# gyhandy/Neural-Sim-NeRF

Hardware: AMD Instinct MI355X
Metric: Mray-samples/sec at 400x400, 64+128 samples, 8x256 MLP (higher is better)
Workload: dtype f16x2

## Files before the change

### neural_sim_nerf_amd/csrc/nsr_kernels.hip

```cpp
#include <hip/hip_runtime.h>
#include <stdint.h>
#include "nsr_device.h"

#if !defined(NSR_UNIT_F32) && !defined(NSR_UNIT_H2) && !defined(NSR_UNIT_B3) && !defined(NSR_UNIT_X16)
#define NSR_UNIT_F32 1
#define NSR_UNIT_H2 1
#define NSR_UNIT_B3 1
#define NSR_UNIT_X16 1
#endif
#ifndef NSR_UNIT_F32
#define NSR_UNIT_F32 0
#endif
#ifndef NSR_UNIT_H2
#define NSR_UNIT_H2 0
#endif
#ifndef NSR_UNIT_B3
#define NSR_UNIT_B3 0
#endif
#ifndef NSR_UNIT_X16
#define NSR_UNIT_X16 0
#endif
#define NSR_CAT_(a, b) a##b
#define NSR_CAT(a, b) NSR_CAT_(a, b)

// ... 70 lines not shown
  rg.pslot = __builtin_amdgcn_readfirstlane(rg.pslot);
  rg.pphase = __builtin_amdgcn_readfirstlane(rg.pphase);
  rg.cslot = __builtin_amdgcn_readfirstlane(rg.cslot);
  rg.pnet_off = __builtin_amdgcn_readfirstlane(rg.pnet_off);
  rg.pnet_next = __builtin_amdgcn_readfirstlane(rg.pnet_next);
}

#ifndef NSR_H2_SCHED
#define NSR_H2_SCHED 3
#endif
constexpr int kH2RingLag = NSR_H2_SCHED == 3 ? 1 : 0;
template <int NS = kRingSlots, int SLABS = kStreamSlabs, int SLABS_BWD = SLABS, int LAG = 0>
__device__ __forceinline__ void ring_start(Ring& rg, f32x4 (&A0)[4], int lane) {
#pragma unroll 1
  for (int s = 0; s < NS - LAG; ++s) ring_issue<NS, SLABS, SLABS_BWD>(rg);
  asm volatile("s_waitcnt vmcnt(%0)" ::"n"(4 * (NS - LAG - 1)) : "memory");
  __builtin_amdgcn_s_barrier();
  const char* p = rg.smem + rg.cslot * kSlabBytes + lane * 16;
#pragma unroll
  for (int c = 0; c < 4; ++c) A0[c] = *(const f32x4*)(p + c * 1024);
}

template <int U>
__device__ __forceinline__ void ring_load_quarter(const Ring& rg, f32x4 (&A)[4], int lane) {
  const char* p = rg.smem + rg.cslot * kSlabBytes + U * kStepBytes + lane * 16;
#pragma unroll
  for (int c = 0; c < 4; ++c) A[c] = *(const f32x4*)(p + c * 1024);
}

template <int NS = kRingSlots>
__device__ __forceinline__ void ring_advance(Ring& rg, f32x4 (&A)[4], int lane) {
  asm volatile("s_waitcnt vmcnt(%0) lgkmcnt(0)" ::"n"(4 * (NS - 2)) : "memory");
#ifndef NSR_EXP_NOBARRIER
  __builtin_amdgcn_s_barrier();
#endif
  rg.cslot = (rg.cslot + 1 == NS) ? 0 : rg.cslot + 1;
  const char* p = rg.smem + rg.cslot * kSlabBytes + lane * 16;
#pragma unroll
  for (int c = 0; c < 4; ++c) A[c] = *(const f32x4*)(p + c * 1024);
}

#define NSR_MFMA(a, b, c) __builtin_amdgcn_mfma_f32_32x32x2f32((a), (b), (c), 0, 0, 0)
__device__ __forceinline__ f32x16 mfma_op(float a, float b, f32x16 c) { return __builtin_amdgcn_mfma_f32_32x32x2f32(a, b, c, 0, 0, 0); }
__device__ __forceinline__ f32x4 mfma_op(float a, float b, f32x4 c) { return __builtin_amdgcn_mfma_f32_16x16x4f32(a, b, c, 0, 0, 0); }

template <int NMO, int KK0, int KK1, bool ZERO = false, int NACC, typename BOp, typename AccT>
__device__ __forceinline__ void consume(const f32x4 (&A)[4], int step, BOp bop, AccT (&acc)[NACC]) {
#pragma unroll
  for (int kk = KK0; kk < KK1; ++kk)
#pragma unroll
    for (int c = 0; c < 4; ++c) {
      const int n = 4 * step + c, tq = n / NMO, mo = n % NMO;
      if (ZERO && tq == 0 && kk == 0) acc[mo] = mfma_op(A[c][kk], bop(4 * tq + kk), AccT{0});
      else acc[mo] = mfma_op(A[c][kk], bop(4 * tq + kk), acc[mo]);
    }
}

#define NSR_PIN() __builtin_amdgcn_sched_barrier(0)
#define NSR_SGB(mask, n) __builtin_amdgcn_sched_group_barrier((mask), (n), 0)
#define NSR_MASK_VALU 0x002
#define NSR_MASK_SALU 0x004
#define NSR_MASK_MFMA 0x008
#define NSR_MASK_VMEM 0x010
#define NSR_MASK_DSRD 0x100
template <int N_MFMA>
__device__ __forceinline__ void step_pattern() {
#pragma unroll
  for (int i = 0; i < N_MFMA; ++i) {
    NSR_SGB(NSR_MASK_MFMA, 1);
    NSR_SGB(NSR_MASK_DSRD, 1);
    NSR_SGB(NSR_MASK_VALU, 2);
  }
}
template <int N_MFMA>
__device__ __forceinline__ void step_pattern_dma() {
#pragma unroll
  for (int i = 0; i < N_MFMA; ++i) {
    NSR_SGB(NSR_MASK_MFMA, 1);
    NSR_SGB(NSR_MASK_DSRD, 1);
    NSR_SGB(NSR_MASK_VMEM, 1);
    NSR_SGB(NSR_MASK_SALU, 3);
    NSR_SGB(NSR_MASK_VALU, 2);
  }
}

template <int NMO, int NTQ, int NS = kRingSlots, bool ZERO = false, int NACC, typename BOp, typename AccT>
__device__ __forceinline__ void seg(Ring& rg, f32x4 (&A0)[4], f32x4 (&A1)[4], BOp bop, AccT (&acc)[NACC],
                                    int lane) {
  static_assert((NMO * NTQ) % 16 == 0, "a segment is a whole number of slabs");
#pragma unroll
  for (int s = 0; s < NMO * NTQ / 4; s += 4) {
    NSR_PIN(); ring_load_quarter<1>(rg, A1, lane); consume<NMO, 0, 4, ZERO>(A0, s, bop, acc);     step_pattern<16>();
    NSR_PIN(); ring_load_quarter<2>(rg, A0, lane); consume<NMO, 0, 4, ZERO>(A1, s + 1, bop, acc); step_pattern<16>();
    NSR_PIN(); ring_load_quarter<3>(rg, A1, lane); consume<NMO, 0, 4, ZERO>(A0, s + 2, bop, acc); step_pattern<16>();
    NSR_PIN(); consume<NMO, 0, 1, ZERO>(A1, s + 3, bop, acc);
    NSR_PIN(); ring_advance<NS>(rg, A0, lane);
    ring_issue<NS>(rg); consume<NMO, 1, 4, ZERO>(A1, s + 3, bop, acc); step_pattern_dma<12>();
    NSR_PIN();
  }
}

template <int NG>
struct BRegs16 {
  const f32x16 (&v)[NG];
  __device__ __forceinline__ float operator()(int t) const { return v[t >> 4][t & 15]; }
};
template <int N>
struct BArr {
  const float (&v)[N];
  __device__ __forceinline__ float operator()(int t) const { return v[t]; }
};
struct BViews {
  const f32x16 (&v)[8];
  const float (&ed)[16];
  __device__ __forceinline__ float operator()(int t) const { return t < 128 ? v[(t & 127) >> 4][t & 15] : ed[t & 15]; }
};

__device__ __forceinline__ int aux_half(int lane) { return opaque_v((lane >> 5) * 4); }

template <int NMO>
__device__ __forceinline__ void load_bias(const float* bias, int h4 , f32x16 (&acc)[NMO]) {
#pragma unroll
  for (int mo = 0; mo < NMO; ++mo)
#pragma unroll
    for (int rq = 0; rq < 4; ++rq) {
      f32x4 v = *(const f32x4*)(bias + (mo * 4 + rq) * 8 + h4);
      acc[mo][rq * 4 + 0] = v[0];
      acc[mo][rq * 4 + 1] = v[1];
      acc[mo][rq * 4 + 2] = v[2];
      acc[mo][rq * 4 + 3] = v[3];
    }
}

#include "nsr_b3.inc"
#include "nsr_h2.inc"

constexpr int kMlpF32 = 0;
constexpr int kMlpB3 = 1;
constexpr int kMlpH2 = 2;

template <int NMO>
__device__ __forceinline__ uint4 relu_mask(const f32x16 (&acc)[NMO]) {
  unsigned w[4] = {0u, 0u, 0u, 0u};
#pragma unroll
  for (int mo = 0; mo < NMO; ++mo)
#pragma unroll
    for (int r = 0; r < 16; ++r) {
      const int on = max(__float_as_int(acc[mo][r]), 0) - 1;
      w[mo >> 1] = __builtin_amdgcn_alignbit(w[mo >> 1], (unsigned)on, 31);
    }
  return make_uint4(w[0], w[1], w[2], w[3]);
}

__device__ __forceinline__ float enc_trig(float a, int k) {
  const double kMagic = 6755399441055744.0;
  const double t = (double)a * 0.63661977236758134308;
  const double tm = t + kMagic;
  const int n = __double2loint(tm) + k;
  const double f = t - (tm - kMagic);
  const float r = (float)(f * 1.57079632679489661923);
  const float z = r * r;
  float ps = __builtin_fmaf(-1.9515295891e-4f, z, 8.3321608736e-3f);
  ps = __builtin_fmaf(ps, z, -1.6666654611e-1f);
  ps = __builtin_fmaf(ps * z, r, r);
  float pc = __builtin_fmaf(2.443315711809948e-5f, z, -1.388731625493765e-3f);
  pc = __builtin_fmaf(pc, z, 4.166664568298827e-2f);
  pc = __builtin_fmaf(pc * z, z, __builtin_fmaf(-0.5f, z, 1.0f));
  const float v = (n & 1) ? pc : ps;
  return __uint_as_float(__float_as_uint(v) ^ ((unsigned)(n & 2) << 30));
}

__device__ __forceinline__ float enc_domain(float x, int nfreq) {
  return __builtin_fabsf(x) < ldexpf(1.0f, 25 - nfreq) ? x : __builtin_nanf("");
}

__device__ __forceinline__ float enc_poison(float px, float py, float pz, float vx, float vy, float vz) {
  const float a = (enc_domain(px, kMultires) * 0.0f + enc_domain(py, kMultires) * 0.0f) + enc_domain(pz, kMultires) * 0.0f;
  const float b = (enc_domain(vx, kMultiresViews) * 0.0f + enc_domain(vy, kMultiresViews) * 0.0f) +
                  enc_domain(vz, kMultiresViews) * 0.0f;
  return __builtin_fabsf(a + b);
}

template <bool CAPTURE, int MODE = kMlpF32>
__device__ __forceinline__ void mlp_pass(Ring& rg, const float* aux, f32x4 (&A0)[4], f32x4 (&A1)[4], int lane,
                                         float px, float py, float pz, float vx, float vy, float vz,
                                         float (&raw)[4], uint4* mask_dst = nullptr , int mask_tid = 0,
                                         long long* tp = nullptr ) {
#ifdef NSR_PHASE_TIMING
  long long tpl = clock64();
#define NSR_TP(i) do { if (tp) { const long long t_ = clock64(); tp[i] += t_ - tpl; tpl = t_; } } while (0)
#else
#define NSR_TP(i) do { } while (0)
#endif
  const int h = lane >> 5;
  const int h4 = aux_half(lane);
  const float poison = enc_poison(px, py, pz, vx, vy, vz);
  float e[32];
  float ed[16];
  {
    const float p[3] = {px, py, pz};
    const float v[3] = {vx, vy, vz};
#pragma unroll
    for (int L = 0; L < kMultires; ++L)
#pragma unroll
      for (int ax = 0; ax < 3; ++ax) e[3 * L + ax] = enc_trig(enc_domain(p[ax], kMultires) * (float)(1 << L), h);
#pragma unroll
    for (int L = 0; L < kMultiresViews; ++L)
#pragma unroll
      for (int ax = 0; ax < 3; ++ax) ed[3 * L + ax] = enc_trig(enc_domain(v[ax], kMultiresViews) * (float)(1 << L), h);
    e[30] = h ? pz : px;
    e[31] = h ? 0.0f : py;
    ed[12] = h ? vz : vx;
    ed[13] = h ? 0.0f : vy;
    ed[14] = 0.0f;
    ed[15] = 0.0f;
  }

  f32x16 acc[8];
  f32x16 in[8];
  auto enc_src = [&](int kb, int i) { return e[(8 * kb + i) & 31]; };
  auto in_src = [&](int kb, int i) { return in[(kb >> 1) & 7][8 * (kb & 1) + i]; };
  constexpr bool B3 = MODE == kMlpB3;
  constexpr bool H2M = MODE == kMlpH2;
  float amax = 0.0f;
  const float* h2s = aux + kAuxH2Scale;
#if NSR_H2_SCHED == 3 && !defined(NSR_EXP_H2_NOFRAG) && !defined(NSR_EXP_H2_HALFBARRIER) && !defined(NSR_EXP_H2_NOSPLIT)
  constexpr bool TAIL = H2M && !CAPTURE;
#else
  constexpr bool TAIL = false;
#endif
  static_assert(kAuxBiasV == kAuxBias + 9 * 256, "the views layer's bias follows feature_linear's: 'bias of layer L + 1' for L = 8");
  NSR_TP(0);
  load_bias<8>(aux + kAuxBias, h4, acc);
  NSR_TP(2);
  if constexpr (B3) gemm_b3<8, 2>(rg, A0, A1, enc_src, acc, lane);
  else if constexpr (TAIL)
    gemm_h2_tail<4>(rg, A0, A1, enc_src, H2Scale{{h2s[0], 0.0f}, 4}, acc, lane, amax, H2Tail{acc, in, 0, h2_lds_base(aux + kAuxBias + 256, h4)});
  else if constexpr (H2M) gemm_h2<8, 4>(rg, A0, A1, enc_src, H2Scale{{h2s[0], 0.0f}, 4}, acc, lane, amax);
  else seg<8, 8>(rg, A0, A1, BArr<32>{e}, acc, lane);
  NSR_TP(1);
  if (CAPTURE) mask_dst[mask_tid] = relu_mask<8>(acc);
  if constexpr (!TAIL) {
#pragma unroll
    for (int mo = 0; mo < 8; ++mo) in[mo] = relu16(acc[mo]);
  }

  float alpha_part = 0.0f;
#pragma unroll 1
  for (int L = 1; L <= 8; ++L) {
    if constexpr (!TAIL) load_bias<8>(aux + kAuxBias + L * 256, h4, acc);
    NSR_TP(2);
    if (L == 5) {
      if constexpr (B3) gemm_b3<8, 2>(rg, A0, A1, enc_src, acc, lane);
      else if constexpr (H2M) gemm_h2<8, 4>(rg, A0, A1, enc_src, H2Scale{{h2s[9], 0.0f}, 4}, acc, lane, amax);
      else seg<8, 8>(rg, A0, A1, BArr<32>{e}, acc, lane);
      NSR_TP(1);
    }
    if (L == 8) {
      const float* wa = aux + kAuxWAlpha;
#pragma unroll
      for (int tq = 0; tq < 32; ++tq) {
        f32x4 w = *(const f32x4*)(wa + tq * 8 + h4);
#pragma unroll
        for (int kk = 0; kk < 4; ++kk)
          alpha_part = __builtin_fmaf(w[kk], in[(4 * tq + kk) >> 4][(4 * tq + kk) & 15], alpha_part);
      }
    }
    if constexpr (B3) gemm_b3<8, 8>(rg, A0, A1, in_src, acc, lane);
    else if constexpr (TAIL)
      gemm_h2_tail<16>(rg, A0, A1, in_src, H2Scale{{h2s[L], 0.0f}, 16}, acc, lane, amax,
                       H2Tail{acc, in, (L == 8) ? (int)0x80000000 : 0, h2_lds_base(aux + kAuxBias + (L + 1) * 256, h4)});
    else if constexpr (H2M) gemm_h2<8, 16>(rg, A0, A1, in_src, H2Scale{{h2s[L], 0.0f}, 16}, acc, lane, amax);
    else seg<8, 32>(rg, A0, A1, BRegs16<8>{in}, acc, lane);
    NSR_TP(1);
    if (CAPTURE && L < 8) mask_dst[L * 256 + mask_tid] = relu_mask<8>(acc);
    if constexpr (!TAIL) {
      const int thr = (L == 8) ? (int)0x80000000 : 0;
#pragma unroll
      for (int mo = 0; mo < 8; ++mo) in[mo] = clamp_bits16(acc[mo], thr);
    }
  }

  f32x16 av[4];
  if constexpr (TAIL) {
#pragma unroll
    for (int mo = 0; mo < 4; ++mo) av[mo] = acc[mo];
  } else {
    load_bias<4>(aux + kAuxBiasV, h4, av);
  }
  NSR_TP(2);
  if constexpr (B3) {
    auto v_src = [&](int kb, int i) {
      return kb < 16 ? in[(kb >> 1) & 7][8 * (kb & 1) + i] : (kb < 18 ? ed[(8 * (kb - 16) + i) & 15] : 0.0f);
    };
    gemm_b3<4, 5>(rg, A0, A1, v_src, av, lane);
  } else if constexpr (H2M) {
    auto v_src = [&](int kb, int i) { return kb < 16 ? in[(kb >> 1) & 7][8 * (kb & 1) + i] : ed[(8 * (kb - 16) + i) & 15]; };
    gemm_h2<4, 18>(rg, A0, A1, v_src, H2Scale{{h2s[10], h2s[11]}, 16}, av, lane, amax);
  } else {
    seg<4, 36>(rg, A0, A1, BViews{in, ed}, av, lane);
  }
  NSR_TP(1);
  if (CAPTURE) mask_dst[8 * 256 + mask_tid] = relu_mask<4>(av);

  float part[4] = {0.0f, 0.0f, 0.0f, alpha_part};
  if constexpr (H2M) {
    const float ov = amax > kH2Max ? __builtin_nanf("") : 0.0f;
    part[0] = part[1] = part[2] = ov;
    part[3] = alpha_part + ov;
  }
#pragma unroll
  for (int c = 0; c < 3; ++c) {
    const float* wr = aux + kAuxWRgb + c * 128;
#pragma unroll
    for (int mo = 0; mo < 4; ++mo)
#pragma unroll
      for (int rq = 0; rq < 4; ++rq) {
        f32x4 w = *(const f32x4*)(wr + (mo * 4 + rq) * 8 + h4);
#pragma unroll
        for (int ri = 0; ri < 4; ++ri)
          part[c] = __builtin_fmaf(w[ri], fmaxf(av[mo][rq * 4 + ri], 0.0f), part[c]);
      }
  }
#pragma unroll
  for (int c = 0; c < 4; ++c) {
    float other = __shfl_xor(part[c], 32);
    float lo_half = h ? other : part[c];
    float hi_half = h ? part[c] : other;
    raw[c] = ((lo_half + hi_half) + aux[(c < 3) ? (kAuxBRgb + c) : kAuxBAlpha]) + poison;
  }
  NSR_TP(3);
#undef NSR_TP
}

template <int NSS, int NFS>
struct ItemStateT {
  static constexpr int kNS = NSS, kNF = NFS;
  float tcoarse[NSS];
  float ufine[128];
  float ray[2][16];
  float zc[2][NSS];
  float rawc[2][NSS][4];
  float w0[2][NSS];
  float cdf[2][NSS];
  float zs[2][128];
  float zf[2][NFS];
  float rawf[2][NFS][4];
  float alpha[2][NFS];
  float wf[2][NFS];
  float tf[2][NFS];
  float om[2][NFS];
  float bwd_scratch[2][NFS][2];
  float psum[2][NFS / 32][12];
  float gnorm[2];
  float res[2][8];
};
typedef ItemStateT<64, 192> ItemState;
typedef ItemStateT<128, 256> ItemStateBig;
static_assert(sizeof(ItemState) == 23048, "the YCB-V layout is part of the shipped kernels' LDS budget");
template <int NS> struct ItemStateFor { typedef ItemState type; };
template <> struct ItemStateFor<128> { typedef ItemStateBig type; };

__device__ __forceinline__ float sigmoidf_(float x) { return 1.0f / (1.0f + expf(-x)); }

template <int S, int R = 2, int STRIDE = S, typename ST>
__device__ __forceinline__ void composite(ST& st, const float* z, float* raw, float* wout, float* tout, int tid,
                                          const float* noise = nullptr ,
                                          long long row0 = 0, int valid = R) {
  static_assert(S % 8 == 0, "scan is unrolled by 8");
// ... 325 lines not shown
    __syncthreads();
  }
}

__device__ __forceinline__ void gen_ray(const float* __restrict__ c2w, float fx, float fy, float cx, float cy,
                                        int row, int col, float (&o)[3], float (&d)[3]) {
  const float dx = ((float)col - cx) / fx;
  const float dy = -(((float)row - cy) / fy);
  const float dz = -1.0f;
#pragma unroll
  for (int a = 0; a < 3; ++a) {
    d[a] = ((dx * c2w[a * 4 + 0]) + (dy * c2w[a * 4 + 1])) + (dz * c2w[a * 4 + 2]);
    o[a] = c2w[a * 4 + 3];
  }
}

struct RenderArgs {
  const float* nets;
  long long net_stride;
  const float* aux[2];
  const float* tcoarse;
  const float* ufine;
  const float* rays_o;
  const float* rays_d;
  const float* c2w;
  float fx, fy, cx, cy;
  int H, W;
  long long n_rays;
  float near_, far_;
  int fine;
  int camera;
  int white_bkgd;
  int lindisp;
  float *rgb, *disp, *acc, *rgb0, *disp0, *acc0, *z_std;
  float *dbg_w0, *dbg_zs, *dbg_zf, *dbg_raw0, *dbg_raw;
  long long* dbg_inds;
  float* zf_scratch;
  int chunk;
  unsigned* sched_flags;
  unsigned* status;
  int super_lg;
  int spin_max;
  unsigned epoch;
  unsigned* epoch_counter;
  unsigned long long* work_counter;
  const float* viewdirs;
  const float* t_rand;
  const float* u_rays;
  const float* noise0;
  const float* noise1;
  const float* near_rays;
  const float* far_rays;
  unsigned long long* ovf_items;
  unsigned* ovf_stat;
  unsigned ovf_cap;
  const unsigned long long* item_list;
  const unsigned* item_count;
  unsigned item_cap;
};

__device__ __forceinline__ void load_aux(char* smem, const RenderArgs& a, int tid) {
  float* dst = (float*)(smem + kLdsAux);
  for (int i = tid; i < kAuxFloats; i += 256) {
    dst[i] = a.aux[0][i];
    dst[kAuxFloats + i] = a.aux[1][i];
  }
}

#if NSR_UNIT_F32
__global__ void k_set_args(const RenderArgs a, RenderArgs* dst) {
  *dst = a;
  *a.work_counter = 0ull;
  if (a.ovf_stat) a.ovf_stat[0] = 0u;
  if (a.epoch_counter) dst->epoch = *a.epoch_counter = *a.epoch_counter % 4094u + 1u;
}
#endif

constexpr long long kItemMask = (1ll << 62) - 1;
__device__ __forceinline__ long long queue_next_item(const RenderArgs& q) {
  const unsigned long long v = atomicAdd(q.work_counter, 1ull);
  if (q.item_list) {
    unsigned n = *q.item_count;
    n = n < q.item_cap ? n : q.item_cap;
    return v < (unsigned long long)n ? (long long)q.item_list[v] : -1ll;
  }
  return v < (unsigned long long)((q.n_rays + 1) >> 1) ? (long long)(v | (3ull << 62)) : -1ll;
}
__device__ __forceinline__ long long queue_item_of(const RenderArgs& q, unsigned long long v) {
  if (q.item_list) {
    unsigned n = *q.item_count;
    n = n < q.item_cap ? n : q.item_cap;
    return v < (unsigned long long)n ? (long long)q.item_list[v] : -1ll;
  }
  return v < (unsigned long long)((q.n_rays + 1) >> 1) ? (long long)(v | (3ull << 62)) : -1ll;
}
__device__ __forceinline__ long long queue_items(const RenderArgs& q) {
  if (q.item_list) { const unsigned n = *q.item_count; return (long long)(n < q.item_cap ? n : q.item_cap); }
  return (q.n_rays + 1) >> 1;
}
__device__ __forceinline__ void range_mark(int* ovf, float chk, int lane) {
#ifndef NSR_EXP_NO_RANGE
  if (chk != chk && lane < 32) atomicAdd(ovf, 1);
#endif
}
__device__ __forceinline__ unsigned range_report(const RenderArgs& a, int* ovf, long long item, int valid) {
#ifdef NSR_EXP_NO_RANGE
  return 0u;
#endif
  const int p0 = ovf[0], p1 = valid == 2 ? ovf[1] : 0;
  if ((p0 | p1) != 0 && a.ovf_stat) {
    const unsigned long long mask = (p0 ? 1ull : 0ull) | (p1 ? 2ull : 0ull);
    const unsigned n = atomicAdd(a.ovf_stat, 1u);
    atomicAdd(a.ovf_stat + 1, (unsigned)(p0 + p1));
    if (n < a.ovf_cap) {
      a.ovf_items[n] = (unsigned long long)item | (mask << 62);
      atomicAdd(a.ovf_stat + 2, (unsigned)((p0 != 0) + (p1 != 0)));
    } else {
      atomicAdd(a.ovf_stat + 3, 1u);
      return (unsigned)mask;
    }
  }
  return 0u;
}
__device__ __forceinline__ void range_poison(const RenderArgs& a, long long ray0, unsigned mask) {
  const float qn = __builtin_nanf("");
  for (int r = 0; r < 2; ++r) {
    if (!((mask >> r) & 1u)) continue;
    const long long rr = ray0 + r;
    float* const v3[2] = {a.rgb, a.rgb0};
    float* const v1[5] = {a.disp, a.acc, a.disp0, a.acc0, a.z_std};
    for (int k = 0; k < 2; ++k) if (v3[k]) { v3[k][rr * 3] = qn; v3[k][rr * 3 + 1] = qn; v3[k][rr * 3 + 2] = qn; }
    for (int k = 0; k < 5; ++k) if (v1[k]) v1[k][rr] = qn;
  }
}

__device__ __forceinline__ void wave_lds_sync() {
  __builtin_amdgcn_fence(__ATOMIC_RELEASE, "wavefront");
  __builtin_amdgcn_wave_barrier();
  __builtin_amdgcn_fence(__ATOMIC_ACQUIRE, "wavefront");
}
__device__ __forceinline__ void lds_barrier() { asm volatile("s_waitcnt lgkmcnt(0)\n\ts_barrier" ::: "memory"); }

template <typename ST>
struct FwdItemExtra {
  float om[2][ST::kNS];
  float tf[2][ST::kNS];
  float zf[2][ST::kNF];
  float ray[2][16];
  float res[2][8];
  long long pend;
  long long next;
};

template <int S>
__device__ __forceinline__ void composite_wave(const float* ry, const float* zr, float* q, float* wr, float* tr, float* omr,
                                               int lane, const float* noise ,
                                               float (&res)[6]) {
  static_assert(S % 8 == 0, "scan is unrolled by 8");
  constexpr int K = (S + 63) / 64;
  float al[K];
#pragma unroll
  for (int k = 0; k < K; ++k) {
    const int i = lane + 64 * k;
    al[k] = 0.0f;
    if (i < S) {
      float dist = (i < S - 1) ? (zr[i + 1] - zr[i]) : 1e10f;
      dist = dist * ry[11];
      if (noise) q[i * 4 + 3] = q[i * 4 + 3] + noise[i];
      const float sigma = fmaxf(q[i * 4 + 3], 0.0f);
      const float a = 1.0f - expf(-sigma * dist);
      al[k] = a;
      omr[i] = (1.0f - a) + 1e-10f;
      q[i * 4 + 0] = sigmoidf_(q[i * 4 + 0]);
      q[i * 4 + 1] = sigmoidf_(q[i * 4 + 1]);
      q[i * 4 + 2] = sigmoidf_(q[i * 4 + 2]);
    }
  }
  wave_lds_sync();
  if (lane == 0) {
    double T = 1.0;
#pragma unroll 1
    for (int i0 = 0; i0 < S; i0 += 8) {
      double f[8];
#pragma unroll
      for (int k = 0; k < 8; ++k) f[k] = (double)omr[i0 + k];
#pragma unroll
      for (int k = 0; k < 8; ++k) {
        tr[i0 + k] = (float)T;
        T = T * f[k];
      }
    }
  }
  wave_lds_sync();
  float cr = 0.f, cg = 0.f, cb = 0.f, depth = 0.f, acc = 0.f;
#pragma unroll
  for (int k = 0; k < K; ++k) {
    const int i = lane + 64 * k;
    if (i < S) {
      const float w = al[k] * tr[i];
      wr[i] = w;
      cr = cr + w * q[i * 4 + 0];
      cg = cg + w * q[i * 4 + 1];
      cb = cb + w * q[i * 4 + 2];
      depth = depth + w * zr[i];
      acc = acc + w;
    }
  }
#pragma unroll
  for (int m = 32; m >= 1; m >>= 1) {
    cr += __shfl_xor(cr, m); cg += __shfl_xor(cg, m); cb += __shfl_xor(cb, m);
    depth += __shfl_xor(depth, m); acc += __shfl_xor(acc, m);
  }
  const float qd = depth / acc;
  float disp;
  if (qd != qd) disp = qd;
  else disp = 1.0f / fmaxf(1e-10f, qd);
  if (ry[12] != 0.0f) {
    const float bg = 1.0f - acc;
    cr = cr + bg; cg = cg + bg; cb = cb + bg;
  }
  res[0] = cr; res[1] = cg; res[2] = cb; res[3] = disp; res[4] = acc; res[5] = depth;
  wave_lds_sync();
}

template <int NI, int NS>
__device__ __forceinline__ void sample_pdf_wave(const float* w, const float* zc, float* x, float* pdf, float* cdf, float* zs,
                                                const float* u ,
                                                int64_t* inds_out , int lane) {
  constexpr int NW = NS - 2, NC = NS - 1;
  constexpr int NVEC = NW / 8, SILP = NVEC / 4;
  constexpr int KW = (NW + 63) / 64;
  float xv[KW];
#pragma unroll
  for (int k = 0; k < KW; ++k) {
    const int i = lane + 64 * k;
    xv[k] = 0.0f;
    if (i < NW) { xv[k] = w[i] + 1e-5f; x[i] = xv[k]; }
  }
  wave_lds_sync();
  const int j = lane & 7;
  float lj;
  if constexpr (NS == 64) {
    const float p0 = ((x[j] + x[32 + j]) + x[40 + j]) + x[48 + j];
    lj = ((p0 + x[8 + j]) + x[16 + j]) + x[24 + j];
  } else {
    float ps[4] = {0.0f, 0.0f, 0.0f, 0.0f};
#pragma unroll
    for (int i = 0; i < SILP; ++i)
#pragma unroll
      for (int k = 0; k < 4; ++k) ps[k] = ps[k] + x[(i * 4 + k) * 8 + j];
#pragma unroll
    for (int v = SILP * 4; v < NVEC; ++v) ps[0] = ps[0] + x[v * 8 + j];
    lj = ((ps[0] + ps[1]) + ps[2]) + ps[3];
  }
  float total = 0.0f;
#pragma unroll
  for (int i = NVEC * 8; i < NW; ++i) total = total + x[i];
#pragma unroll
  for (int jj = 0; jj < 8; ++jj) total = total + __shfl(lj, jj);
#pragma unroll
  for (int k = 0; k < KW; ++k) {
    const int i = lane + 64 * k;
    if (i < NW) pdf[i] = xv[k] / total;
  }
  wave_lds_sync();
  if (lane == 0) {
    double run = 0.0;
    cdf[0] = 0.0f;
#pragma unroll 1
    for (int i0 = 0; i0 < NVEC * 8; i0 += 8) {
      double f[8];
#pragma unroll
      for (int k = 0; k < 8; ++k) f[k] = (double)pdf[i0 + k];
#pragma unroll
      for (int k = 0; k < 8; ++k) { run = run + f[k]; cdf[i0 + k + 1] = (float)run; }
    }
#pragma unroll
    for (int i = NVEC * 8; i < NW; ++i) { run = run + (double)pdf[i]; cdf[i + 1] = (float)run; }
  }
  wave_lds_sync();
#pragma unroll
  for (int kk = 0; kk < (NI + 63) / 64; ++kk) {
    const int k = lane + 64 * kk;
    if (k < NI) {
      const float uu = u[k];
      int lo = 0, hi = NC;
      while (lo < hi) {
        const int mid = (lo + hi) >> 1;
        if (cdf[NSR_IDX(mid, NC)] <= uu) lo = mid + 1; else hi = mid;
      }
      const int ind = lo;
      const int below = NSR_IDX(max(ind - 1, 0), NC);
      const int above = NSR_IDX(min(ind, NC - 1), NC);
      const float c0 = cdf[below], c1 = cdf[above];
      const float b0 = 0.5f * (zc[below + 1] + zc[below]), b1 = 0.5f * (zc[above + 1] + zc[above]);
      float denom = c1 - c0;
      if (denom < 1e-5f) denom = 1.0f;
      const float t = (uu - c0) / denom;
      zs[NSR_IDX(k, 128)] = b0 + t * (b1 - b0);
      if (inds_out) inds_out[k] = (int64_t)ind;
    }
  }
  wave_lds_sync();
}

template <int NI, int NS>
__device__ __forceinline__ void merge_wave(const float* zc, const float* zs, float* zf, int lane) {
  constexpr int NF = NS + NI;
  constexpr bool kPow2 = (NI & (NI - 1)) == 0 && (NS & (NS - 1)) == 0;
  constexpr int K = (NF + 63) / 64;
  int bad = 0;
#pragma unroll
  for (int kk = 0; kk < K; ++kk) {
    const int k = lane + 64 * kk;
    if (k < NS - 1) bad |= !(zc[k] <= zc[k + 1]);
    else if (k >= NS && k < NF - 1) bad |= !(zs[k - NS] <= zs[k - NS + 1]);
  }
  const bool any_bad = __builtin_amdgcn_ballot_w64(bad != 0) != 0;
  if (!any_bad) {
#pragma unroll
    for (int kk = 0; kk < K; ++kk) {
      const int k = lane + 64 * kk;
      if (k < NS) {
        const float x = zc[k];
        int lb = 0;
        if constexpr (kPow2) {
#pragma unroll
          for (int sft = NI / 2; sft > 0; sft >>= 1) lb += (zs[lb + sft - 1] < x) ? sft : 0;
          lb += (zs[lb] < x) ? 1 : 0;
        } else {
          int hi = NI;
          while (lb < hi) { const int mid = (lb + hi) >> 1; if (zs[NSR_IDX(mid, NI)] < x) lb = mid + 1; else hi = mid; }
        }
        zf[NSR_IDX(k + lb, NF)] = x;
      } else if (k < NF) {
        const float x = zs[k - NS];
        int ub = 0;
        if constexpr (kPow2) {
#pragma unroll
          for (int sft = NS / 2; sft > 0; sft >>= 1) ub += (zc[ub + sft - 1] <= x) ? sft : 0;
          ub += (zc[ub] <= x) ? 1 : 0;
        } else {
          int hi = NS;
          while (ub < hi) { const int mid = (ub + hi) >> 1; if (zc[NSR_IDX(mid, NS)] <= x) ub = mid + 1; else hi = mid; }
        }
        zf[NSR_IDX((k - NS) + ub, NF)] = x;
      }
    }
  } else {
#pragma unroll 1
    for (int kk = 0; kk < K; ++kk) {
      const int k = lane + 64 * kk;
      if (k < NF) {
        const float x = (k < NS) ? zc[k] : zs[k - NS];
        int rank = 0;
        for (int jx = 0; jx < NS; ++jx) {
          const float y = zc[jx];
          rank += (y < x) || (y == x && jx < k);
        }
        for (int jx = 0; jx < NI; ++jx) {
          const float y = zs[jx];
          rank += (y < x) || (y == x && (jx + NS) < k);
        }
        zf[NSR_IDX(rank, NF)] = x;
      }
    }
  }
  wave_lds_sync();
}

#ifdef NSR_PHASE_TIMING
#define NSR_T(i) do { if (threadIdx.x == 0) { const long long t_ = clock64(); tacc[i] += t_ - tlast; tlast = t_; } } while (0)
#else
#define NSR_T(i) do { } while (0)
#endif

template <int MODE, int NI = 128, int NS = 64>
__device__ __forceinline__ void render32_body(const RenderArgs* __restrict__ ap, char* smem) {
  constexpr bool B3 = MODE == kMlpB3;
  constexpr int NF = NS + NI;
  constexpr int NP = (2 * NF + 127) / 128;
  constexpr int NPC = (2 * NS + 127) / 128;
  constexpr int LNS = NS == 32 ? 5 : (NS == 64 ? 6 : 7);
  typedef typename ItemStateFor<NS>::type ST;
  static_assert((NS == 32 || NS == 64 || NS == 128) && NF % 32 == 0 && NS <= ST::kNS && NF <= ST::kNF,
                "a wave's points belong to one ray; the item state holds kNS coarse / kNF fine samples per ray");
  const RenderArgs& a_setup = *ap;
#ifdef NSR_PHASE_TIMING
  long long tacc[8] = {0, 0, 0, 0, 0, 0, 0, 0};
  long long tpass[4] = {0, 0, 0, 0};
  long long tlast = clock64();
#define NSR_TPASS tpass
#else
#define NSR_TPASS nullptr
#endif
  const int tid0 = threadIdx.x;
  const int lane = tid0 & 63;
  const int wave = __builtin_amdgcn_readfirstlane(tid0 >> 6);
  const int j = lane & 31;
  ST& st = *(ST*)(smem + kLdsState);

  const long long n_rays = a_setup.n_rays;
  if ((long long)blockIdx.x >= queue_items(a_setup)) return;
  const int fine = a_setup.fine;
  typedef FwdItemExtra<ST> XT;
  static_assert(offsetof(ST, res) - offsetof(ST, bwd_scratch) >= sizeof(XT) && offsetof(ST, bwd_scratch) % 8 == 0 &&
                offsetof(XT, pend) % 8 == 0, "the forward scratch lives in the item state's backward scratch");
  XT& xs = *(XT*)&st.bwd_scratch[0][0][0];

  Ring rg;
  ring_init(rg, smem, a_setup.nets, a_setup.net_stride, fine ? NPC + NP : NPC, wave, lane);
  rg.pn0 = NPC; rg.pn1 = NPC + NP;

  f32x4 A0[4], A1[4];
  if constexpr (B3) ring_start<kRingSlots, kStreamSlabsB3, kStreamSlabsB3Bwd>(rg, A0, lane);
  else if constexpr (MODE == kMlpH2) ring_start<kRingSlots, kStreamSlabs, kStreamSlabs, kH2RingLag>(rg, A0, lane);
  else ring_start(rg, A0, lane);

  load_aux(smem, a_setup, tid0);
  if (tid0 < NS) st.tcoarse[tid0] = a_setup.tcoarse[tid0];
  if (tid0 < NI) st.ufine[tid0] = a_setup.ufine[tid0];
  if (tid0 == 0) xs.pend = -1ll;
  __syncthreads();
  const float* aux_c = (const float*)(smem + kLdsAux);

  long long* item_slot = (long long*)&st.ray[0][14];
  auto next_item = [&]() -> long long {
    if (opaque_v(tid0) == 0) *item_slot = queue_next_item(*opaque_s(ap));
    lds_barrier();
    const long long v = uniform64(*item_slot);
    lds_barrier();
    return v;
  };

  auto fine_wave = [&](long long pk, int pp, int r) {
    const RenderArgs& a = *opaque_s(ap);
    const long long ray0 = (pk & kItemMask) * 2;
    const int valid = (ray0 + 1 < n_rays) ? 2 : 1;
    const int wmask = (int)((unsigned long long)pk >> 62) & (valid == 2 ? 3 : 1);
    const float* ry = pp ? xs.ray[r] : st.ray[r];
    const float* zr = pp ? xs.zf[r] : st.zf[r];
    float* q = &st.rawf[r][0][0];
    if (a.dbg_raw && ((wmask >> r) & 1)) {
      for (int idx = lane; idx < NF * 4; idx += 64) a.dbg_raw[(ray0 + r) * (NF * 4) + idx] = q[idx];
      wave_lds_sync();
    }
    float res[6];
    composite_wave<NF>(ry, zr, q, st.wf[r], st.tf[r], st.om[r], lane,
                       a.noise1 ? a.noise1 + (ray0 + (r < valid ? r : 0)) * NF : nullptr, res);
    if (lane == 0) {
#pragma unroll
      for (int c = 0; c < 6; ++c) st.res[r][c] = res[c];
    }
  };
  auto fine_out = [&](long long pk, int pp) {
    const RenderArgs& a = *opaque_s(ap);
    const int tid = opaque_v(tid0);
    const long long item = pk & kItemMask;
    const long long ray0 = item * 2;
    const int valid = (ray0 + 1 < n_rays) ? 2 : 1;
    const int wmask = (int)((unsigned long long)pk >> 62) & (valid == 2 ? 3 : 1);
    if (tid < 16 && ((wmask >> (tid >> 3)) & 1)) {
      const int r = tid >> 3, c = tid & 7;
      const long long rr = ray0 + r;
      const float v = st.res[r][c];
      if (c < 3) { if (a.rgb) a.rgb[rr * 3 + c] = v; }
      else if (c == 3) { if (a.disp) a.disp[rr] = v; }
      else if (c == 4) { if (a.acc) a.acc[rr] = v; }
    }
    if (MODE == kMlpH2 && tid == 0) {
      int* povf = (int*)(pp ? &xs.ray[1][14] : &st.ray[1][14]);
      if (const unsigned m = range_report(a, povf, item, valid)) range_poison(a, ray0, m);
    }
  };

  long long packed = next_item();
  int pass = 0;
  int par = 0;
#pragma unroll 1
  while (packed != -1ll) {
    const long long item = packed & kItemMask;
    const long long ray0 = item * 2;
    const int valid = (ray0 + 1 < n_rays) ? 2 : 1;
    const int wmask = (int)((unsigned long long)packed >> 62) & (valid == 2 ? 3 : 1);
    auto wr = [&](int r) { return ((wmask >> r) & 1) != 0; };
    float (*const ray)[16] = par ? xs.ray : st.ray;
    float* const zf = par ? &xs.zf[0][0] : &st.zf[0][0];
    int* const ovf = (int*)&ray[1][14];
    if (pass == 0) {
      const RenderArgs& a = *opaque_s(ap);
      const int tid = opaque_v(tid0);
      const float near_ = a.near_, far_ = a.far_;
      if (tid < 2) {
        const long long rr = ray0 + (tid < valid ? tid : 0);
        float o[3], d[3];
        if (a.camera) {
          const long long hw = (long long)a.H * a.W;
          const long long v = rr / hw;
          const int pix = (int)(rr - v * hw);
          gen_ray(a.c2w + v * 12, a.fx, a.fy, a.cx, a.cy, pix / a.W, pix % a.W, o, d);
        } else {
#pragma unroll
          for (int c = 0; c < 3; ++c) { o[c] = a.rays_o[rr * 3 + c]; d[c] = a.rays_d[rr * 3 + c]; }
        }
        const float nrm = sqrtf(((d[0] * d[0]) + (d[1] * d[1])) + (d[2] * d[2]));
        const float* vd = a.camera ? nullptr : a.viewdirs;
#pragma unroll
        for (int c = 0; c < 3; ++c) {
          ray[tid][c] = o[c]; ray[tid][3 + c] = d[c];
          ray[tid][6 + c] = vd ? vd[rr * 3 + c] : d[c] / nrm;
        }
        ray[tid][9] = a.near_rays ? a.near_rays[rr] : near_;
        ray[tid][10] = a.near_rays ? a.far_rays[rr] : far_;
        ray[tid][11] = nrm;
        ray[tid][12] = a.white_bkgd ? 1.0f : 0.0f;
      }
      if (MODE == kMlpH2 && (tid == 64 || tid == 65)) ovf[tid - 64] = 0;
      if (tid < 2 * NS) {
        const int r = tid >> LNS, i = tid & (NS - 1);
        const float t = st.tcoarse[i];
        const long long rb = ray0 + (r < valid ? r : 0);
        st.zc[r][i] = coarse_z(a.near_rays ? a.near_rays[rb] : near_, a.near_rays ? a.far_rays[rb] : far_, t, a.lindisp);
      }
      lds_barrier();
      if (a.t_rand) perturb_coarse_z<NS>(st, a.t_rand, ray0, valid, tid);
      NSR_T(0);
    }

    {
      int r, i;
      const float* zsrc;
      float* dst;
      bool real = true;
      if ((NPC == 1) ? (pass == 0) : (pass < NPC)) {
        if constexpr (NS == 64) {
          r = wave >> 1; i = 32 * (wave & 1) + j;
        } else {
          int q0 = 128 * pass + 32 * wave;
          if (2 * NS % 128 != 0 && q0 >= 2 * NS) { q0 = 2 * NS - 32; real = false; }
          r = q0 >> LNS; i = (q0 & (NS - 1)) + j;
        }
        zsrc = &st.zc[r][i]; dst = st.rawc[r][i];
      } else {
        int q0 = 128 * (pass - NPC) + 32 * wave;
        if (2 * NF % 128 != 0 && q0 >= 2 * NF) { q0 = 2 * NF - 32; real = false; }
        r = q0 / NF; i = q0 - r * NF + j;
        zsrc = &zf[r * ST::kNF + i]; dst = st.rawf[r][i];
      }
      const float z = *zsrc;
      const float* ry = ray[r];
      float raw[4];
      mlp_pass<false, MODE>(rg, aux_c + (((NPC == 1) ? (pass == 0) : (pass < NPC)) ? 0 : kAuxFloats), A0, A1, lane, ry[0] + ry[3] * z, ry[1] + ry[4] * z,
               ry[2] + ry[5] * z, ry[6], ry[7], ry[8], raw, nullptr, 0, NSR_TPASS);
      if (lane < 32 && real) *(f32x4*)dst = f32x4{raw[0], raw[1], raw[2], raw[3]};
      if constexpr (MODE == kMlpH2) { if (real) range_mark(ovf + r, (raw[0] + raw[1]) + (raw[2] + raw[3]), lane); }
    }
    NSR_T(1);

    const RenderArgs& a = *opaque_s(ap);
    const int tid = opaque_v(tid0);
    if (NPC > 1 && pass < NPC - 1) {
      ++pass;
    } else if ((NPC == 1) ? (pass == 0) : (pass < NPC)) {
      lds_barrier();
      const long long pend = fine ? uniform64(xs.pend) : -1ll;
      const bool puller = fine && tid == 192;
      unsigned long long ticket = 0ull;
      if (puller) ticket = atomicAdd(a.work_counter, 1ull);
      if (wave < 2) {
        const int r = wave;
        float* q = &st.rawc[r][0][0];
        if (a.dbg_raw0 && wr(r)) {
          for (int idx = lane; idx < NS * 4; idx += 64) a.dbg_raw0[(ray0 + r) * (NS * 4) + idx] = q[idx];
          wave_lds_sync();
        }
        float res[6];
        composite_wave<NS>(ray[r], st.zc[r], q, st.w0[r], xs.tf[r], xs.om[r], lane,
                           a.noise0 ? a.noise0 + (ray0 + (r < valid ? r : 0)) * NS : nullptr, res);
        if (lane == 0) {
#pragma unroll
          for (int c = 0; c < 6; ++c) xs.res[r][c] = res[c];
        }
        if (a.dbg_w0 && wr(r))
          for (int idx = lane; idx < NS; idx += 64) a.dbg_w0[(ray0 + r) * NS + idx] = st.w0[r][idx];
        NSR_T(2);
        if (fine) {
#ifdef NSR_PHASE_TIMING
          int64_t* inds = nullptr;
#else
          int64_t* inds = (int64_t*)a.dbg_inds;
#endif
          sample_pdf_wave<NI, NS>(&st.w0[r][1], st.zc[r], xs.tf[r], xs.om[r], st.cdf[r], st.zs[r],
                                  a.u_rays ? a.u_rays + (ray0 + (r < valid ? r : 0)) * 128 : st.ufine,
                                  (inds && wr(r)) ? inds + (ray0 + r) * NI : nullptr, lane);
          NSR_T(3);
          const float sd = zstd_wave<NI>(st, r, lane);
          if (lane == 0 && wr(r) && a.z_std) a.z_std[ray0 + r] = sd;
          if (a.dbg_zs && wr(r))
            for (int k = lane; k < NI; k += 64) a.dbg_zs[(ray0 + r) * NI + k] = st.zs[r][k];
          NSR_T(4);
          merge_wave<NI, NS>(st.zc[r], st.zs[r], zf + r * ST::kNF, lane);
          if (a.dbg_zf && wr(r))
            for (int k = lane; k < NF; k += 64) a.dbg_zf[(ray0 + r) * NF + k] = zf[r * ST::kNF + k];
          NSR_T(5);
        }
      } else if (pend != -1ll) {
#ifdef NSR_PHASE_TIMING
        const long long t0_ = clock64();
#endif
        fine_wave(pend, par ^ 1, wave - 2);
#ifdef NSR_PHASE_TIMING
        if (threadIdx.x == 128) tacc[7] += clock64() - t0_;
#endif
      }
      if (puller) xs.next = queue_item_of(a, ticket);
      lds_barrier();
      if (pend != -1ll) fine_out(pend, par ^ 1);
      if (tid < 16 && wr(tid >> 3)) {
        const int r = tid >> 3, c = tid & 7;
        const long long rr = ray0 + r;
        const float v = xs.res[r][c];
        float* rgb_dst = fine ? a.rgb0 : a.rgb;
        float* disp_dst = fine ? a.disp0 : a.disp;
        float* acc_dst = fine ? a.acc0 : a.acc;
        if (c < 3) { if (rgb_dst) rgb_dst[rr * 3 + c] = v; }
        else if (c == 3) { if (disp_dst) disp_dst[rr] = v; }
        else if (c == 4) { if (acc_dst) acc_dst[rr] = v; }
      }
      NSR_T(6);
      if (!fine) {
        if (MODE == kMlpH2 && tid == 0) { if (const unsigned m = range_report(a, ovf, item, valid)) range_poison(a, ray0, m); }
        if constexpr (NPC > 1) pass = 0;
        packed = next_item(); continue;
      }
      pass = NPC;
    } else if (pass < NPC + NP - 1) {
      ++pass;
    } else {
      if (tid == 0) xs.pend = packed;
      pass = 0;
      par ^= 1;
      packed = uniform64(xs.next);
    }
  }
  if (fine) {
    lds_barrier();
    const long long pend = uniform64(xs.pend);
    if (pend != -1ll) {
      if (wave < 2) fine_wave(pend, par ^ 1, wave);
      lds_barrier();
      fine_out(pend, par ^ 1);
    }
    NSR_T(6);
  }
  asm volatile("s_waitcnt vmcnt(0)" ::: "memory");
#ifdef NSR_PHASE_TIMING
  if (tid0 == 128 && a_setup.dbg_raw == nullptr && a_setup.dbg_inds) a_setup.dbg_inds[blockIdx.x * 8 + 7] = tacc[7];
  if (tid0 == 0 && a_setup.dbg_raw == nullptr && a_setup.dbg_inds)
    for (int i = 0; i < 7; ++i) a_setup.dbg_inds[blockIdx.x * 8 + i] = tacc[i];
  if (tid0 == 0 && a_setup.dbg_raw == nullptr && a_setup.dbg_inds)
    for (int i = 0; i < 4; ++i) a_setup.dbg_inds[(long long)gridDim.x * 8 + blockIdx.x * 4 + i] = tpass[i];
#endif
#undef NSR_TPASS
}

#define NSR_RENDER_KERNEL_1(NAME, ...)                                                               \
  __global__ void __launch_bounds__(256, 1) NAME(const RenderArgs* __restrict__ ap) {                \
    extern __shared__ __attribute__((aligned(16))) char smem[];                                      \
    render32_body<__VA_ARGS__>(ap, smem);                                                            \
  }
#define NSR_RENDER_KERNEL_0(NAME, ...) __global__ void __launch_bounds__(256, 1) NAME(const RenderArgs* __restrict__ ap);
#define NSR_RENDER_KERNEL(UNIT, NAME, ...) NSR_CAT(NSR_RENDER_KERNEL_, UNIT)(NAME, __VA_ARGS__)
NSR_RENDER_KERNEL(NSR_UNIT_F32, k_render, kMlpF32)
NSR_RENDER_KERNEL(NSR_UNIT_B3, k_render_b3, kMlpB3)
NSR_RENDER_KERNEL(NSR_UNIT_H2, k_render_h2, kMlpH2)
NSR_RENDER_KERNEL(NSR_UNIT_H2, k_render_h2_n64, kMlpH2, 64)
NSR_RENDER_KERNEL(NSR_UNIT_H2, k_render_h2_n32, kMlpH2, 32)
NSR_RENDER_KERNEL(NSR_UNIT_B3, k_render_b3_n64, kMlpB3, 64)
NSR_RENDER_KERNEL(NSR_UNIT_B3, k_render_b3_n32, kMlpB3, 32)
NSR_RENDER_KERNEL(NSR_UNIT_H2, k_render_h2_n96, kMlpH2, 96, 64)
NSR_RENDER_KERNEL(NSR_UNIT_B3, k_render_b3_n96, kMlpB3, 96, 64)
NSR_RENDER_KERNEL(NSR_UNIT_H2, k_render_h2_c32_n64, kMlpH2, 64, 32)
NSR_RENDER_KERNEL(NSR_UNIT_B3, k_render_b3_c32_n64, kMlpB3, 64, 32)
NSR_RENDER_KERNEL(NSR_UNIT_H2, k_render_h2_c128_n128, kMlpH2, 128, 128)
NSR_RENDER_KERNEL(NSR_UNIT_B3, k_render_b3_c128_n128, kMlpB3, 128, 128)
#undef NSR_RENDER_KERNEL
#undef NSR_RENDER_KERNEL_0
#undef NSR_RENDER_KERNEL_1

__device__ __forceinline__ f32x16 apply_mask(f32x16 x, unsigned word, int shift) {
  f32x16 r;
#pragma unroll
  for (int i = 0; i < 16; ++i)
    r[i] = ((word >> (31 - (shift + i))) & 1u) ? 0.0f : x[i];
  return r;
}

template <int NFREQ>
__device__ __forceinline__ void embed_bwd(const float (&x)[3], const float* G , int h,
                                          float (&out)[3]) {
  out[0] = h ? 0.0f : G[3 * NFREQ];
  out[1] = h ? 0.0f : G[3 * NFREQ + 1];
  out[2] = h ? G[3 * NFREQ] : 0.0f;
#pragma unroll
  for (int L = 0; L < NFREQ; ++L)
#pragma unroll
// ... 1797 lines not shown
```

Baseline: 282.2.

## Halve positional-encoding trig work with permlane swaps and stage view-dir encodings in LDS

In the non-capture forward pass, each half-wave now runs the range reduction and sin/cos polynomials once per frequency, each half covering a different set of frequencies. The sin and cos results are exchanged between half-waves with permlane32_swap, where before both halves computed every frequency and kept only one of sin or cos. The view-direction encoding is constant per ray, so spare threads compute it once per item into an LDS image (reusing the alpha buffer), and every MLP pass reads it with 16-byte loads. This removes redundant double-precision reduction and polynomial work per sample, at the cost of cross-lane swaps, extra LDS traffic and reuse of an existing LDS region.

```diff
diff --git a/neural_sim_nerf_amd/csrc/nsr_kernels.hip b/neural_sim_nerf_amd/csrc/nsr_kernels.hip
--- a/neural_sim_nerf_amd/csrc/nsr_kernels.hip
+++ b/neural_sim_nerf_amd/csrc/nsr_kernels.hip
@@ -246,7 +246,8 @@
   return make_uint4(w[0], w[1], w[2], w[3]);
 }
 
-__device__ __forceinline__ float enc_trig(float a, int k) {
+struct EncRed { int n; float ps, pc; };
+__device__ __forceinline__ EncRed enc_reduce(float a, int k = 0) {
   const double kMagic = 6755399441055744.0;
   const double t = (double)a * 0.63661977236758134308;
   const double tm = t + kMagic;
@@ -260,8 +261,20 @@
   float pc = __builtin_fmaf(2.443315711809948e-5f, z, -1.388731625493765e-3f);
   pc = __builtin_fmaf(pc, z, 4.166664568298827e-2f);
   pc = __builtin_fmaf(pc * z, z, __builtin_fmaf(-0.5f, z, 1.0f));
-  const float v = (n & 1) ? pc : ps;
+  return EncRed{n, ps, pc};
+}
+__device__ __forceinline__ float enc_pick(const EncRed& q, int k = 0) {
+  const int n = q.n + k;
+  const float v = (n & 1) ? q.pc : q.ps;
   return __uint_as_float(__float_as_uint(v) ^ ((unsigned)(n & 2) << 30));
+}
+__device__ __forceinline__ float enc_trig(float a, int k) { return enc_pick(enc_reduce(a, k)); }
+
+__device__ __forceinline__ void enc_pair(float a, float& lo, float& hi) {
+  const EncRed q = enc_reduce(a);
+  const auto x = __builtin_amdgcn_permlane32_swap(__float_as_uint(enc_pick(q, 0)), __float_as_uint(enc_pick(q, 1)), false, false);
+  lo = __uint_as_float(x[0]);
+  hi = __uint_as_float(x[1]);
 }
 
 __device__ __forceinline__ float enc_domain(float x, int nfreq) {
@@ -275,11 +288,13 @@
   return __builtin_fabsf(a + b);
 }
 
-template <bool CAPTURE, int MODE = kMlpF32>
+template <bool CAPTURE, int MODE = kMlpF32, bool DIMG = false>
 __device__ __forceinline__ void mlp_pass(Ring& rg, const float* aux, f32x4 (&A0)[4], f32x4 (&A1)[4], int lane,
                                          float px, float py, float pz, float vx, float vy, float vz,
                                          float (&raw)[4], uint4* mask_dst = nullptr , int mask_tid = 0,
-                                         long long* tp = nullptr ) {
+                                         long long* tp = nullptr ,
+                                         const float* dimg = nullptr) {
+  static_assert(!(CAPTURE && DIMG), "the input-gradient kernels keep their encodings");
 #ifdef NSR_PHASE_TIMING
   long long tpl = clock64();
 #define NSR_TP(i) do { if (tp) { const long long t_ = clock64(); tp[i] += t_ - tpl; tpl = t_; } } while (0)
@@ -291,7 +306,7 @@
   const float poison = enc_poison(px, py, pz, vx, vy, vz);
   float e[32];
   float ed[16];
-  {
+  if constexpr (CAPTURE) {
     const float p[3] = {px, py, pz};
     const float v[3] = {vx, vy, vz};
 #pragma unroll
@@ -308,7 +323,40 @@
     ed[13] = h ? 0.0f : vy;
     ed[14] = 0.0f;
     ed[15] = 0.0f;
-  }
+  } else {
+    static_assert(kMultires == 10 && kMultiresViews == 4, "half of the frequencies per half-wave");
+    const float fp = h ? 32.0f : 1.0f;
+    const float p[3] = {enc_domain(px, kMultires) * fp, enc_domain(py, kMultires) * fp, enc_domain(pz, kMultires) * fp};
+#pragma unroll
+    for (int k = 0; k < 15; ++k) enc_pair(p[k % 3] * (float)(1 << (k / 3)), e[k], e[k + 15]);
+    e[30] = h ? pz : px;
+    e[31] = h ? 0.0f : py;
+    if constexpr (DIMG) {
+#pragma unroll
+      for (int q = 0; q < 4; ++q) {
+        const f32x4 w = *(const f32x4*)(dimg + 16 * h + 4 * q);
+#pragma unroll
+        for (int i = 0; i < 4; ++i) ed[4 * q + i] = w[i];
+      }
+    } else {
+      const float fv = h ? 4.0f : 1.0f;
+      const float v[3] = {enc_domain(vx, kMultiresViews) * fv, enc_domain(vy, kMultiresViews) * fv, enc_domain(vz, kMultiresViews) * fv};
+#pragma unroll
+      for (int k = 0; k < 6; ++k) enc_pair(v[k % 3] * (float)(1 << (k / 3)), ed[k], ed[k + 6]);
+      ed[12] = h ? vz : vx;
+      ed[13] = h ? 0.0f : vy;
+      ed[14] = 0.0f;
+      ed[15] = 0.0f;
+    }
+  }
+#ifdef NSR_PHASE_TIMING
+#pragma unroll
+  for (int i = 0; i < 32; i += 8)
+    asm volatile("" :: "v"(e[i]), "v"(e[i + 1]), "v"(e[i + 2]), "v"(e[i + 3]), "v"(e[i + 4]), "v"(e[i + 5]), "v"(e[i + 6]), "v"(e[i + 7]));
+#pragma unroll
+  for (int i = 0; i < 16; i += 8)
+    asm volatile("" :: "v"(ed[i]), "v"(ed[i + 1]), "v"(ed[i + 2]), "v"(ed[i + 3]), "v"(ed[i + 4]), "v"(ed[i + 5]), "v"(ed[i + 6]), "v"(ed[i + 7]));
+#endif
 
   f32x16 acc[8];
   f32x16 in[8];
@@ -940,6 +988,18 @@
   long long next;
 };
 
+__device__ __forceinline__ void stage_dir_image(float* img, const float (&v)[3], int t) {
+  const int L = t / 3, ax = t - 3 * L;
+  const float x = ax == 0 ? v[0] : (ax == 1 ? v[1] : v[2]);
+  const EncRed q = enc_reduce(enc_domain(x, kMultiresViews) * (float)(1 << L));
+  img[t] = enc_pick(q, 0);
+  img[16 + t] = enc_pick(q, 1);
+  if (t == 0) {
+    *(f32x4*)(img + 12) = f32x4{v[0], v[1], 0.0f, 0.0f};
+    *(f32x4*)(img + 28) = f32x4{v[2], 0.0f, 0.0f, 0.0f};
+  }
+}
+
 template <int S>
 __device__ __forceinline__ void composite_wave(const float* ry, const float* zr, float* q, float* wr, float* tr, float* omr,
                                                int lane, const float* noise ,
@@ -1195,6 +1255,8 @@
   static_assert(offsetof(ST, res) - offsetof(ST, bwd_scratch) >= sizeof(XT) && offsetof(ST, bwd_scratch) % 8 == 0 &&
                 offsetof(XT, pend) % 8 == 0, "the forward scratch lives in the item state's backward scratch");
   XT& xs = *(XT*)&st.bwd_scratch[0][0][0];
+  static_assert((kLdsState + offsetof(ST, alpha)) % 16 == 0 && sizeof(st.alpha) >= 2 * 2 * 2 * 16 * sizeof(float),
+                "the direction image is read with 16-byte LDS loads");
 
   Ring rg;
   ring_init(rg, smem, a_setup.nets, a_setup.net_stride, fine ? NPC + NP : NPC, wave, lane);
@@ -1275,12 +1337,16 @@
     float (*const ray)[16] = par ? xs.ray : st.ray;
     float* const zf = par ? &xs.zf[0][0] : &st.zf[0][0];
     int* const ovf = (int*)&ray[1][14];
+    float* const dimg = &st.alpha[0][0] + 64 * par;
     if (pass == 0) {
       const RenderArgs& a = *opaque_s(ap);
       const int tid = opaque_v(tid0);
       const float near_ = a.near_, far_ = a.far_;
-      if (tid < 2) {
-        const long long rr = ray0 + (tid < valid ? tid : 0);
+      const int dt = tid - 128;
+      const bool dtask = dt >= 0 && dt < 24;
+      if (tid < 2 || dtask) {
+        const int rt = dtask ? (dt >= 12 ? 1 : 0) : tid;
+        const long long rr = ray0 + (rt < valid ? rt : 0);
         float o[3], d[3];
         if (a.camera) {
           const long long hw = (long long)a.H * a.W;
@@ -1293,15 +1359,22 @@
         }
         const float nrm = sqrtf(((d[0] * d[0]) + (d[1] * d[1])) + (d[2] * d[2]));
         const float* vd = a.camera ? nullptr : a.viewdirs;
-#pragma unroll
-        for (int c = 0; c < 3; ++c) {
-          ray[tid][c] = o[c]; ray[tid][3 + c] = d[c];
-          ray[tid][6 + c] = vd ? vd[rr * 3 + c] : d[c] / nrm;
-        }
-        ray[tid][9] = a.near_rays ? a.near_rays[rr] : near_;
-        ray[tid][10] = a.near_rays ? a.far_rays[rr] : far_;
-        ray[tid][11] = nrm;
-        ray[tid][12] = a.white_bkgd ? 1.0f : 0.0f;
+        float vdir[3];
+#pragma unroll
+        for (int c = 0; c < 3; ++c) vdir[c] = vd ? vd[rr * 3 + c] : d[c] / nrm;
+        if (dtask) {
+          stage_dir_image(dimg + rt * 32, vdir, dt - 12 * rt);
+        } else {
+#pragma unroll
+          for (int c = 0; c < 3; ++c) {
+            ray[tid][c] = o[c]; ray[tid][3 + c] = d[c];
+            ray[tid][6 + c] = vdir[c];
+          }
+          ray[tid][9] = a.near_rays ? a.near_rays[rr] : near_;
+          ray[tid][10] = a.near_rays ? a.far_rays[rr] : far_;
+          ray[tid][11] = nrm;
+          ray[tid][12] = a.white_bkgd ? 1.0f : 0.0f;
+        }
       }
       if (MODE == kMlpH2 && (tid == 64 || tid == 65)) ovf[tid - 64] = 0;
       if (tid < 2 * NS) {
@@ -1338,8 +1411,8 @@
       const float z = *zsrc;
       const float* ry = ray[r];
       float raw[4];
-      mlp_pass<false, MODE>(rg, aux_c + (((NPC == 1) ? (pass == 0) : (pass < NPC)) ? 0 : kAuxFloats), A0, A1, lane, ry[0] + ry[3] * z, ry[1] + ry[4] * z,
-               ry[2] + ry[5] * z, ry[6], ry[7], ry[8], raw, nullptr, 0, NSR_TPASS);
+      mlp_pass<false, MODE, true>(rg, aux_c + (((NPC == 1) ? (pass == 0) : (pass < NPC)) ? 0 : kAuxFloats), A0, A1, lane, ry[0] + ry[3] * z, ry[1] + ry[4] * z,
+               ry[2] + ry[5] * z, ry[6], ry[7], ry[8], raw, nullptr, 0, NSR_TPASS, dimg + r * 32);
       if (lane < 32 && real) *(f32x4*)dst = f32x4{raw[0], raw[1], raw[2], raw[3]};
       if constexpr (MODE == kMlpH2) { if (real) range_mark(ovf + r, (raw[0] + raw[1]) + (raw[2] + raw[3]), lane); }
     }
```

Result: no change. 284.2 (median of 6 runs) (+0.7%).
